# nintendops/EPN_PointCloud

Measured on AMD Instinct MI355X. Metric: point-clouds/sec fwd+bwd, ModelNet40 N=1024 A=60, higher is better.
Workload: dtype f32

## Files before the change

epn_pointcloud_amd/csrc/c_api.hip:

```cpp
#include <atomic>
#include <cstdlib>
#include <cstring>
#include <cxxabi.h>

#include "conv_internal.h"

using namespace epn;

static std::atomic<int> g_policy{0};
static bool force_generic() { return g_policy.load(std::memory_order_relaxed) == 1; }

namespace epn {
bool first_layer_on_valu() { return g_policy.load(std::memory_order_relaxed) == 2; }
#ifdef EPN_TUNING
int kernel_policy() { return g_policy.load(std::memory_order_relaxed); }
#else
int kernel_policy() { return 0; }
#endif
}

namespace {
thread_local const void *t_stub = nullptr;
thread_local bool t_stub_aux = true;
}
namespace epn {
void note_kernel(const void *host_stub, bool aux) {
    if (aux && t_stub) return;
    t_stub = host_stub;
    t_stub_aux = aux;
}
}

extern "C" const char *epn_last_kernel(void) {
    static thread_local char out[320];
    out[0] = 0;
    const void *stub = t_stub;
    t_stub = nullptr;
    t_stub_aux = true;
    if (!stub) return out;
    const char *mangled = hipKernelNameRefByPtr(stub, nullptr);
    if (!mangled) return out;
    int status = 0;
    char *dem = abi::__cxa_demangle(mangled, nullptr, nullptr, &status);
    const char *b = (status == 0 && dem) ? dem : mangled;
    if (!std::strncmp(b, "void ", 5)) b += 5;
    static const char anon[] = "(anonymous namespace)::";
    size_t o = 0;
    int depth = 0;
    for (size_t i = 0; b[i] && o + 1 < sizeof(out);) {
        if (!std::strncmp(b + i, anon, sizeof(anon) - 1)) { i += sizeof(anon) - 1; continue; }
        if (b[i] == '<') ++depth;
        else if (b[i] == '>') --depth;
        else if (b[i] == '(' && depth == 0) break;
        out[o++] = b[i++];
    }
    out[o] = 0;
    std::free(dem);
    return out;
}

extern "C" int epn_set_kernel_policy(int policy) {
#ifdef EPN_TUNING
    if (policy != 0 && policy != 1 && policy != 2 && (policy & ~0xff) != 0x100 && (policy & ~0xff) != 0x200 && (policy & ~0xff) != 0x400 && (policy & ~0xff) != 0x800 && (policy & ~0xff) != 0x900) return EPN_EINVAL;
#else
    if (policy != 0 && policy != 1 && policy != 2) return EPN_EINVAL;
#endif
    g_policy.store(policy, std::memory_order_relaxed);
    return 0;
}

static int check_desc(const epn_inter_desc *d) {
    if (!d) return EPN_ENULL;
    if (d->b < 0 || d->p1 < 1 || d->p2 < 0 || d->nn < 1 || d->na < 1 || d->ks < 1 || d->cin < 1 || d->cout < 1)
        return EPN_EINVAL;
    if (d->ks > EPN_KS_GENERIC_MAX) return EPN_EINVAL;
    if (!(d->sigma > 0.f) && !d->dense_w) return EPN_EINVAL;
    if (!d->ball_idx) return EPN_ENULL;
    if (!d->dense_w && (!d->xyz || !d->new_xyz || !d->anchors || !d->kernels)) return EPN_ENULL;
    return 0;
}

static bool use_mfma(const epn_inter_desc *d) { return inter_uses_mfma(d) && !force_generic() && !d->dense_w; }

extern "C" const char *epn_version(void) { return "epn_so3conv 0.5 (gfx950)"; }
extern "C" int epn_abi_version(void) { return EPN_ABI_VERSION; }

extern "C" const char *epn_strerror(int code) {
    switch (code) {
        case 0: return "success";
        case EPN_EINVAL: return "epn: invalid size or unsupported shape";
        case EPN_EWORKSPACE: return "epn: workspace missing or too small";
        case EPN_ENULL: return "epn: required pointer is NULL";
        default: return code > 0 ? hipGetErrorString((hipError_t)code) : "epn: unknown error";
    }
}

extern "C" int epn_inter_is_fused(const epn_inter_desc *d) {
    return d && (use_mfma(d) || (inter_c1_fwd_ok(d) && !force_generic())) ? 1 : 0;
// ... 480 lines not shown
```

epn_pointcloud_amd/csrc/gemm.h:

```cpp
#pragma once
#include "epn_common.h"

namespace epn {

constexpr int GEMM_MAX_PROB = 6;

struct GemmNtProb {
    const void *A, *Bt;
    void *C;
    long long M, lda, ldb, ldc;
    int N, K;
    int tiles_n;
    unsigned tile0;
    unsigned ntile;
    const void *Bp;
    float *stats;
    const float *a_amax, *b_amax;
    unsigned *c_amax;
};
struct GemmNtBatch {
    int nprob;
    unsigned ntiles;
    GemmNtProb p[GEMM_MAX_PROB];
};
// ... 21 lines not shown
        if (rc) return rc;
    }
    return 0;
}

inline unsigned nt_plan_tiles(GemmNtBatch &B, int BM, int BN) {
    for (int i = 1; i < B.nprob; ++i)
        for (int k = i; k > 0 && B.p[k].K > B.p[k - 1].K; --k) {
            const GemmNtProb tmp = B.p[k]; B.p[k] = B.p[k - 1]; B.p[k - 1] = tmp;
        }
    unsigned total = 0;
    for (int i = 0; i < B.nprob; ++i) {
        GemmNtProb &p = B.p[i];
        p.tiles_n = (p.N + BN - 1) / BN;
        p.tile0 = total;
        p.ntile = (unsigned)((p.M + BM - 1) / BM) * p.tiles_n;
        total += i + 1 < B.nprob ? (p.ntile + 7u) & ~7u : p.ntile;
    }
    B.ntiles = total;
    return total;
}

struct GemmTnArgs {
    const void *X, *Y;
    void *C, *part;
    size_t part_bytes;
    long long R, ldx, ldy, ldc;
    int N1, N2;
    unsigned ntiles;
    int tiles_n2, nsplit;
    unsigned block0;
    const void *Xp;
    const float *x_amax, *y_amax;
};
struct GemmTnBatch {
    int nprob;
    unsigned nblocks;
    GemmTnArgs p[GEMM_MAX_PROB];
};

#ifdef __HIPCC__
typedef __attribute__((address_space(3))) void lds_void;
typedef __attribute__((address_space(1))) const void glb_void;
typedef __bf16 bf16x8 __attribute__((ext_vector_type(8)));
typedef __bf16 bf16x4 __attribute__((ext_vector_type(4)));
typedef __bf16 bf16x2 __attribute__((ext_vector_type(2)));
typedef short s16x4 __attribute__((ext_vector_type(4)));
typedef float f32x2 __attribute__((ext_vector_type(2)));
typedef unsigned u32x4 __attribute__((ext_vector_type(4)));

template <typename T> struct ElemOf;
template <> struct ElemOf<float> { static constexpr int PER16 = 4; };
template <> struct ElemOf<__bf16> { static constexpr int PER16 = 8; };

__device__ __forceinline__ void glds16(const void *g, char *lds_wave_base) {
    __builtin_amdgcn_global_load_lds((glb_void *)g, (lds_void *)lds_wave_base, 16, 0, 0);
}

#define EPN_WAVE_UMAX(m_)                                                                       \
    _Pragma("unroll") for (int o = 32; o >= 1; o >>= 1) {                                        \
        const unsigned v = (unsigned)__shfl_xor((int)(m_), o, 64);                               \
        (m_) = v > (m_) ? v : (m_);                                                              \
    }
__device__ __forceinline__ unsigned absmax_finite(unsigned m, unsigned bits) {
    const unsigned a = bits & 0x7fffffffu;
    return (a > m && a < 0x7f800000u) ? a : m;
// ... 181 lines not shown
            const int n = col0 + 32 * j + li;
            if (lj == 0 && n < N) {
                float2 *o = reinterpret_cast<float2 *>(part + (((size_t)(rb >> 5)) * N + n) * 2);
                *o = make_float2(s1, s2);
            }
        }
    }
}
#endif

#ifdef __HIPCC__
template <int TM, int TN, typename TO>
__device__ __forceinline__ void nt_c_amax(const gemm_f32x16 (&acc)[TM][TN], unsigned *__restrict__ out) {
    float mf = 0.0f;
#pragma unroll
    for (int i = 0; i < TM; ++i)
#pragma unroll
        for (int j = 0; j < TN; ++j)
#pragma unroll
            for (int r = 0; r < 16; r += 2) mf = fmaxf(fmaxf(mf, fabsf(acc[i][j][r])), fabsf(acc[i][j][r + 1]));
    if constexpr (sizeof(TO) == 2) mf = (float)(__bf16)mf;
    unsigned m = __builtin_bit_cast(unsigned, mf);
    m = m < 0x7f800000u ? m : 0u;
    EPN_WAVE_UMAX(m)
    if ((threadIdx.x & 63) == 0 && m > __atomic_load_n(out, __ATOMIC_RELAXED)) atomicMax(out, m);
}
#endif

long long f2_nonfinite_take_gemm(bool reset);
long long f2_nonfinite_take_x3(bool reset);
long long f2_nonfinite_take_bwd(bool reset);

int kernel_policy();

int launch_gemm_nt(GemmNtBatch &B, int dtype, int out_dtype, hipStream_t st);
bool gemm_nt_x3_ok(const GemmNtBatch &B);
size_t gemm_nt_x3_workspace(const GemmNtBatch &B);
int launch_gemm_nt_x3(GemmNtBatch &B, void *ws, size_t ws_bytes, hipStream_t st, int npl = 3);
size_t gemm_nt_f2_workspace(const GemmNtBatch &B);
int launch_absmax(const float *src, long long ld, long long rows, long long cols, float *out, hipStream_t st);
int launch_scale_scalar(float *v, float factor, hipStream_t st, unsigned tag = 0);
int launch_absmax_unless_tagged(const float *src, long long n, float *slot, unsigned tag, hipStream_t st);
int launch_gemm_tn(GemmTnArgs &G, int dtype, hipStream_t st);
int launch_gemm_tn_batch(GemmTnBatch &B, int dtype, void *ws, size_t ws_bytes, hipStream_t st);
size_t gemm_tn_batch_workspace(GemmTnBatch &B, int dtype);
void gemm_tn_tile(int dtype, int N1, int N2, int *bn1, int *bn2);
int gemm_tn_splits(int dtype, long long R, int N1, int N2);
int launch_transpose_cast(const void *src, void *dst, int rows, int cols, int src_bf16, int dst_bf16, hipStream_t st);
int launch_cast(const void *src, void *dst, size_t n, int src_bf16, int dst_bf16, hipStream_t st);
int launch_cast_add(const float *src, const void *add_bf16, void *dst_bf16, size_t n, hipStream_t st);

}
```

epn_pointcloud_amd/csrc/gemm_tn.hip:

```cpp
#include "conv_internal.h"
#include "gemm.h"

namespace epn {
namespace {
EPN_F2_SENTINEL_DECL


#ifndef EPN_TN_GROUP_TARGET_BF16
#define EPN_TN_GROUP_TARGET_BF16 768
#endif
#ifndef EPN_TN_GROUP_TARGET_F32
#define EPN_TN_GROUP_TARGET_F32 1024
#endif
#ifndef EPN_TN_SINGLE_TARGET_BF16
#define EPN_TN_SINGLE_TARGET_BF16 512
#endif
#ifndef EPN_TN_SWZ
#define EPN_TN_SWZ 1
#endif
__device__ __forceinline__ int tn_row_swz(int r) { return 2 * ((r & 3) | (((r >> 3) & 1) << 2)); }
template <bool SWZ>
__device__ __forceinline__ int tn_swz_col(int col, int r) {
    if constexpr (!SWZ) return col;
    return (((col >> 3) ^ tn_row_swz(r)) << 3) | (col & 7);
}
#ifndef EPN_TN_WIDE_NSTG
#define EPN_TN_WIDE_NSTG 3
#endif
#ifndef EPN_TN_NARROW_NSTG
#define EPN_TN_NARROW_NSTG 4
#endif
#ifndef EPN_TN_NARROW_STAGE_KB
// ... 9 lines not shown
#define EPN_TN_NARROW_WGS 1
#endif
__device__ __forceinline__ unsigned tn_tile_of(unsigned lb, unsigned ntiles, unsigned nsplit) {
    return epn_xcd_tile(lb, (ntiles * nsplit + 7u) & ~7u);
}

template <int W, int K>
__device__ __forceinline__ void tn_frag_k(const char *p, float (&v)[W][K], int k) {
    static_assert(W == 1 || W == 2 || W == 4, "fragment width");
    if constexpr (W == 4) {
        const f32x4 q = *reinterpret_cast<const f32x4 *>(p);
        v[0][k] = q[0]; v[1][k] = q[1]; v[2][k] = q[2]; v[3][k] = q[3];
    } else if constexpr (W == 2) {
        const f32x2 q = *reinterpret_cast<const f32x2 *>(p);
        v[0][k] = q[0]; v[1][k] = q[1];
    } else {
        v[0][k] = *reinterpret_cast<const float *>(p);
    }
}
template <int W>
__device__ __forceinline__ void tn_frag(const char *p, float (&v)[W]) {
    static_assert(W == 1 || W == 2 || W == 4, "fragment width");
    if constexpr (W == 4) {
        const f32x4 q = *reinterpret_cast<const f32x4 *>(p);
        v[0] = q[0]; v[1] = q[1]; v[2] = q[2]; v[3] = q[3];
    } else if constexpr (W == 2) {
        const f32x2 q = *reinterpret_cast<const f32x2 *>(p);
        v[0] = q[0]; v[1] = q[1];
    } else {
        v[0] = *reinterpret_cast<const float *>(p);
    }
}

template <int WGM, int WGN, int TM, int TN, int BR, int X3 = 0>
__global__ __launch_bounds__(64 * WGM * WGN) void gemm_tn_f32_kernel(GemmTnBatch B) {
    constexpr int NW = WGM * WGN;
    constexpr int BN1 = WGM * TM * 32, BN2 = WGN * TN * 32;
    constexpr int ROWF = BN1 + BN2;
    constexpr int STAGE_B = BR * ROWF * 4;
    constexpr int NI = STAGE_B / 1024;
    constexpr int IPW = (NI + NW - 1) / NW;
    static_assert(STAGE_B % 1024 == 0, "stage must be a whole number of 1 KiB pieces");
    __shared__ __attribute__((aligned(1024))) char smem[2 * STAGE_B];

    const int lane = threadIdx.x & 63;
    const int wave = __builtin_amdgcn_readfirstlane(threadIdx.x >> 6);
    int pi = 0;
#pragma unroll
    for (int i = 1; i < GEMM_MAX_PROB; ++i)
        if (i < B.nprob && blockIdx.x >= B.p[i].block0) pi = i;
    const GemmTnArgs &G = B.p[pi];
    const unsigned tile = tn_tile_of(blockIdx.x - G.block0, G.ntiles, (unsigned)G.nsplit) % G.ntiles;
    const unsigned split = tn_tile_of(blockIdx.x - G.block0, G.ntiles, (unsigned)G.nsplit) / G.ntiles;
    if (split >= (unsigned)G.nsplit) return;
    const int n1_0 = (int)(tile / G.tiles_n2) * BN1, n2_0 = (int)(tile % G.tiles_n2) * BN2;
    const long long nchunk = G.R / BR;
    const long long c0 = nchunk * split / G.nsplit, c1 = nchunk * (split + 1) / G.nsplit;
    const int nk = (int)(c1 - c0);
    const float *__restrict__ X = static_cast<const float *>(G.X);
    const float *__restrict__ Y = static_cast<const float *>(G.Y);

    const float *src[IPW];
    long long sstep[IPW];
#pragma unroll
    for (int i = 0; i < IPW; ++i) {
        const int q = wave + i * NW;
// ... 91 lines not shown
                    const int g0 = (i * (NGRP - 1)) / IPW;
                    const int g1 = g0 + 1 < NGRP ? g0 + 1 : NGRP - 1;
                    if ((g0 == s && wpar == 0) || (g1 == s && wpar != 0)) stage_one((kt + 1) & 1, i);
                }
            }
            __builtin_amdgcn_sched_barrier(0);
#pragma unroll
            for (int i = 0; i < TM; ++i)
#pragma unroll
                for (int j = 0; j < TN; ++j)
                    acc[i][j] = __builtin_amdgcn_mfma_f32_32x32x2f32(a[s & 1][i], b[s & 1][j], acc[i][j], 0, 0, 0);
        }
    }

    if constexpr (X3 == 2) {
        const float ux = f2_inverse(x_scale), uy = f2_inverse(y_scale);
        EPN_F2_CHECK(f2_unscale(acc, ux, uy));
    }
    float *__restrict__ C = G.nsplit > 1 ? static_cast<float *>(G.part) + (size_t)split * G.N1 * G.N2
                                         : static_cast<float *>(G.C);
    const long long ldc = G.nsplit > 1 ? G.N2 : G.ldc;
    if (n1_0 + BN1 <= G.N1 && n2_0 + BN2 <= G.N2 && (long long)BN1 * ldc < (1LL << 30)) {
        float *__restrict__ cw = C + (size_t)(n1_0 + wm * TM * 32) * ldc + (n2_0 + wn * TN * 32);
        const unsigned ld = (unsigned)ldc;
        const unsigned lane_off = (unsigned)(TM * 4 * lj) * ld + TN * li;
#pragma unroll
        for (int i = 0; i < TM; ++i)
#pragma unroll
            for (int r = 0; r < 16; ++r) {
                const unsigned o = lane_off + (unsigned)(TM * ((r & 3) + 8 * (r >> 2)) + i) * ld;
#pragma unroll
                for (int j = 0; j < TN; ++j) cw[o + j] = acc[i][j][r];
            }
        return;
    }
#pragma unroll
    for (int i = 0; i < TM; ++i)
#pragma unroll
        for (int r = 0; r < 16; ++r) {
            const int ri = (r & 3) + 8 * (r >> 2) + 4 * lj;
            const int n1 = n1_0 + wm * TM * 32 + TM * ri + i;
            const int n2 = n2_0 + wn * TN * 32 + TN * li;
            if (n1 < G.N1) {
#pragma unroll
                for (int j = 0; j < TN; ++j)
                    if (n2 + j < G.N2) C[(long long)n1 * ldc + n2 + j] = acc[i][j][r];
            }
        }
}

__global__ void split_octets_kernel(const float *__restrict__ X, long long ldx, long long R, int N1, u32x4 *__restrict__ planes) {
    const long long i = (long long)blockIdx.x * blockDim.x + threadIdx.x;
    const long long n = (R >> 3) * N1;
    if (i >= n) return;
    const long long o = i / N1;
    const int c = (int)(i - o * N1);
    float x[8];
#pragma unroll
    for (int k = 0; k < 8; ++k) x[k] = X[(8 * o + k) * ldx + c];
    bf16x8 h, m, l;
    split3(x, h, m, l);
    planes[i] = __builtin_bit_cast(u32x4, h);
    planes[n + i] = __builtin_bit_cast(u32x4, m);
    planes[2 * n + i] = __builtin_bit_cast(u32x4, l);
}

__global__ void split_octets2_kernel(const float *__restrict__ X, long long ldx, long long R, int N1, u32x4 *__restrict__ planes,
                                     const float *__restrict__ amax) {
    const long long i = (long long)blockIdx.x * blockDim.x + threadIdx.x;
    const long long n = (R >> 3) * N1;
    if (i >= n) return;
    const long long o = i / N1;
    const int c = (int)(i - o * N1);
    float x[8];
#pragma unroll
    for (int k = 0; k < 8; ++k) x[k] = X[(8 * o + k) * ldx + c];
    gemm_f16x8 h, l;
    f2_split8(x, f2_scale_of(*amax), h, l);
    planes[i] = __builtin_bit_cast(u32x4, h);
    planes[n + i] = __builtin_bit_cast(u32x4, l);
}
// ... 108 lines not shown
            gemm_f16x8 ah[TM], al[TM], bh[TN], bl[TN];
#pragma unroll
            for (int i = 0; i < TM; ++i) {
                const char *xp = base + (2 * s + lj) * (BN1 * 16) + xo + i * 512;
                ah[i] = *reinterpret_cast<const gemm_f16x8 *>(xp);
                al[i] = *reinterpret_cast<const gemm_f16x8 *>(xp + OCT * BN1 * 16);
            }
#pragma unroll
            for (int j = 0; j < TN; ++j) f2_split8(yb[j], y_scale, bh[j], bl[j]);
            f2_terms(acc, ah, al, bh, bl);
            }
        }
    }

    if constexpr (NPL == 2) {
        const float ux = f2_inverse(f2_scale_of(*G.x_amax)), uy = f2_inverse(y_scale);
        EPN_F2_CHECK(f2_unscale(acc, ux, uy));
    }
    float *__restrict__ C = G.nsplit > 1 ? static_cast<float *>(G.part) + (size_t)split * G.N1 * G.N2
                                         : static_cast<float *>(G.C);
    const long long ldc = G.nsplit > 1 ? G.N2 : G.ldc;
    if (n1_0 + BN1 <= G.N1 && n2_0 + BN2 <= G.N2 && (long long)BN1 * ldc < (1LL << 30)) {
        float *__restrict__ cw = C + (size_t)(n1_0 + wm * TM * 32) * ldc + (n2_0 + wn * TN * 32);
        const unsigned ld = (unsigned)ldc;
        const unsigned lane_off = (unsigned)(4 * lj) * ld + TN * li;
#pragma unroll
        for (int i = 0; i < TM; ++i)
#pragma unroll
            for (int r = 0; r < 16; ++r) {
                const unsigned o = lane_off + (unsigned)(32 * i + (r & 3) + 8 * (r >> 2)) * ld;
#pragma unroll
                for (int j = 0; j < TN; ++j) cw[o + j] = acc[i][j][r];
            }
        return;
    }
#pragma unroll
    for (int i = 0; i < TM; ++i)
#pragma unroll
        for (int r = 0; r < 16; ++r) {
            const int n1 = n1_0 + wm * TM * 32 + 32 * i + (r & 3) + 8 * (r >> 2) + 4 * lj;
            const int n2 = n2_0 + wn * TN * 32 + TN * li;
            if (n1 < G.N1) {
#pragma unroll
                for (int j = 0; j < TN; ++j)
                    if (n2 + j < G.N2) C[(long long)n1 * ldc + n2 + j] = acc[i][j][r];
            }
        }
}

template <int WGM, int WGN, int TM, int TN>
__global__ __launch_bounds__(64 * WGM * WGN) void gemm_tn_bf16_kernel(GemmTnBatch B) {
    constexpr int NW = WGM * WGN;
    constexpr int BR = 32;
    constexpr int BN1 = WGM * TM * 16, BN2 = WGN * TN * 16;
    constexpr int ROWE = BN1 + BN2;
    constexpr int STAGE_B = BR * ROWE * 2;
    constexpr int NI = STAGE_B / 1024;
    constexpr int IPW = (NI + NW - 1) / NW;
    static_assert(STAGE_B % 1024 == 0, "stage must be a whole number of 1 KiB pieces");
    __shared__ __attribute__((aligned(1024))) char smem[2 * STAGE_B];

    const int lane = threadIdx.x & 63;
    const int wave = __builtin_amdgcn_readfirstlane(threadIdx.x >> 6);
    int pi = 0;
#pragma unroll
    for (int i = 1; i < GEMM_MAX_PROB; ++i)
        if (i < B.nprob && blockIdx.x >= B.p[i].block0) pi = i;
    const GemmTnArgs &G = B.p[pi];
    const unsigned tile = tn_tile_of(blockIdx.x - G.block0, G.ntiles, (unsigned)G.nsplit) % G.ntiles;
    const unsigned split = tn_tile_of(blockIdx.x - G.block0, G.ntiles, (unsigned)G.nsplit) / G.ntiles;
    if (split >= (unsigned)G.nsplit) return;
    const int n1_0 = (int)(tile / G.tiles_n2) * BN1, n2_0 = (int)(tile % G.tiles_n2) * BN2;
    const long long nchunk = G.R / BR;
    const long long c0 = nchunk * split / G.nsplit, c1 = nchunk * (split + 1) / G.nsplit;
    const int nk = (int)(c1 - c0);
    const __bf16 *__restrict__ X = static_cast<const __bf16 *>(G.X);
    const __bf16 *__restrict__ Y = static_cast<const __bf16 *>(G.Y);

    constexpr bool SWZ = EPN_TN_SWZ && BN1 % 128 == 0 && BN2 % 128 == 0;
    const __bf16 *src[IPW];
// ... 63 lines not shown
                (__attribute__((address_space(3))) s16x4 *)(base + ((tr_row + 4) * ROWE + col) * 2));
            typedef short s16x8 __attribute__((ext_vector_type(8)));
            const s16x8 v = {lo[0], lo[1], lo[2], lo[3], hi[0], hi[1], hi[2], hi[3]};
            b[j] = __builtin_bit_cast(bf16x8, v);
        }
#pragma unroll
        for (int i = 0; i < TM; ++i)
#pragma unroll
            for (int j = 0; j < TN; ++j) {
                acc[i][j] = __builtin_amdgcn_mfma_f32_16x16x32_bf16(a[i], b[j], acc[i][j], 0, 0, 0);
                if (i == 0 && j == 0) {
                    __builtin_amdgcn_sched_barrier(0);
                    if (kt + 1 < nk) stage((kt + 1) & 1);
                    __builtin_amdgcn_sched_barrier(0);
                }
            }
    }

    float *__restrict__ C = G.nsplit > 1 ? static_cast<float *>(G.part) + (size_t)split * G.N1 * G.N2
                                         : static_cast<float *>(G.C);
    const long long ldc = G.nsplit > 1 ? G.N2 : G.ldc;
    if (n1_0 + BN1 <= G.N1 && n2_0 + BN2 <= G.N2 && (long long)BN1 * ldc < (1LL << 30)) {
        float *__restrict__ cw = C + (size_t)(n1_0 + wm * TM * 16) * ldc + (n2_0 + wn * TN * 16);
        const unsigned ld = (unsigned)ldc;
        const unsigned lane_off = (unsigned)(4 * lg) * ld + li;
#pragma unroll
        for (int i = 0; i < TM; ++i)
#pragma unroll
            for (int r = 0; r < 4; ++r) {
                const unsigned o = lane_off + (unsigned)(i * 16 + r) * ld;
#pragma unroll
                for (int j = 0; j < TN; ++j) cw[o + j * 16] = acc[i][j][r];
            }
        return;
    }
#pragma unroll
    for (int i = 0; i < TM; ++i)
#pragma unroll
        for (int j = 0; j < TN; ++j)
#pragma unroll
            for (int r = 0; r < 4; ++r) {
                const int n1 = n1_0 + (wm * TM + i) * 16 + 4 * lg + r;
                const int n2 = n2_0 + (wn * TN + j) * 16 + li;
                if (n1 < G.N1 && n2 < G.N2) C[(long long)n1 * ldc + n2] = acc[i][j][r];
            }
}

template <int WGM, int WGN, int TM, int TN, int NSTG, int KR>
__global__ __launch_bounds__(64 * WGM * WGN) void gemm_tn_bf16_ring_kernel(GemmTnBatch B) {
    constexpr int NW = WGM * WGN;
    constexpr int BN1 = WGM * TM * 16, BN2 = WGN * TN * 16;
    constexpr int ROWE = BN1 + BN2;
    constexpr int BR = 32 * KR;
    constexpr int STAGE_B = BR * ROWE * 2;
    constexpr int NI = STAGE_B / 1024;
    constexpr int IPW = (NI + NW - 1) / NW;
    static_assert(STAGE_B % 1024 == 0, "stage must be a whole number of 1 KiB pieces");
    static_assert(NSTG >= 3 && NSTG <= 4 && NSTG * STAGE_B <= 160 * 1024, "ring of 3 or 4 stages in LDS");
    static_assert(IPW * (NSTG - 2) <= 63, "vmcnt range");
    __shared__ __attribute__((aligned(1024))) char smem[NSTG * STAGE_B];

    const int lane = threadIdx.x & 63;
    const int wave = __builtin_amdgcn_readfirstlane(threadIdx.x >> 6);
    int pi = 0;
#pragma unroll
    for (int i = 1; i < GEMM_MAX_PROB; ++i)
        if (i < B.nprob && blockIdx.x >= B.p[i].block0) pi = i;
    const GemmTnArgs &G = B.p[pi];
    const unsigned tile = tn_tile_of(blockIdx.x - G.block0, G.ntiles, (unsigned)G.nsplit) % G.ntiles;
    const unsigned split = tn_tile_of(blockIdx.x - G.block0, G.ntiles, (unsigned)G.nsplit) / G.ntiles;
    if (split >= (unsigned)G.nsplit) return;
    const int n1_0 = (int)(tile / G.tiles_n2) * BN1, n2_0 = (int)(tile % G.tiles_n2) * BN2;
    const long long nchunk = G.R / 32;
    const long long c0 = nchunk * split / G.nsplit, c1 = nchunk * (split + 1) / G.nsplit;
    const int nk = (int)(c1 - c0);
    const int nst = (nk + KR - 1) / KR;
    const __bf16 *__restrict__ X = static_cast<const __bf16 *>(G.X);
    const __bf16 *__restrict__ Y = static_cast<const __bf16 *>(G.Y);
// ... 78 lines not shown
                        b[j] = __builtin_bit_cast(bf16x8, v);
                    }
                }
                asm volatile("" : "+v"(lo[TN + i]), "+v"(hi[TN + i]));
                const s16x8 va = {lo[TN + i][0], lo[TN + i][1], lo[TN + i][2], lo[TN + i][3],
                                  hi[TN + i][0], hi[TN + i][1], hi[TN + i][2], hi[TN + i][3]};
                const bf16x8 a = __builtin_bit_cast(bf16x8, va);
#pragma unroll
                for (int j = 0; j < TN; ++j) {
                    acc[i][j] = __builtin_amdgcn_mfma_f32_16x16x32_bf16(a, b[j], acc[i][j], 0, 0, 0);
                    if (ks == 0 && i == 0 && j == 0) {
                        __builtin_amdgcn_sched_barrier(0);
                        if (kt + NSTG - 1 < nst) stage((kt + NSTG - 1) % NSTG);
                        __builtin_amdgcn_sched_barrier(0);
                    }
                }
            }
        }
    }

    float *__restrict__ C = G.nsplit > 1 ? static_cast<float *>(G.part) + (size_t)split * G.N1 * G.N2
                                         : static_cast<float *>(G.C);
    const long long ldc = G.nsplit > 1 ? G.N2 : G.ldc;
#pragma unroll
    for (int i = 0; i < TM; ++i)
#pragma unroll
        for (int j = 0; j < TN; ++j)
#pragma unroll
            for (int r = 0; r < 4; ++r) {
                const int n1 = n1_0 + (wm * TM + i) * 16 + 4 * lg + r;
                const int n2 = n2_0 + (wn * TN + j) * 16 + li;
                if (n1 < G.N1 && n2 < G.N2) C[(long long)n1 * ldc + n2] = acc[i][j][r];
            }
}

__global__ __launch_bounds__(256) void gemm_tn_reduce_kernel(GemmTnBatch B) {
    const GemmTnArgs &G = B.p[blockIdx.y];
    if (G.nsplit <= 1) return;
    const float *__restrict__ part = static_cast<const float *>(G.part);
    float *__restrict__ C = static_cast<float *>(G.C);
    const size_t n = (size_t)G.N1 * G.N2;
    const size_t stride = (size_t)gridDim.x * blockDim.x;
    if ((G.N2 & 3) == 0 && (G.ldc & 3) == 0 && !((uintptr_t)C & 15)) {
        const size_t n4 = n >> 2;
        for (size_t i = (size_t)blockIdx.x * blockDim.x + threadIdx.x; i < n4; i += stride) {
            const f32x4 *p = reinterpret_cast<const f32x4 *>(part) + i;
            f32x4 a[8];
#pragma unroll
            for (int u = 0; u < 8; ++u) a[u] = f32x4{0.f, 0.f, 0.f, 0.f};
            int k = 0;
            for (; k + 8 <= G.nsplit; k += 8)
#pragma unroll
                for (int u = 0; u < 8; ++u) {
                    const f32x4 v = p[(size_t)(k + u) * n4];
                    a[u][0] += v[0]; a[u][1] += v[1]; a[u][2] += v[2]; a[u][3] += v[3];
                }
            for (; k < G.nsplit; ++k) {
                const f32x4 v = p[(size_t)k * n4];
                a[0][0] += v[0]; a[0][1] += v[1]; a[0][2] += v[2]; a[0][3] += v[3];
            }
            f32x4 r;
#pragma unroll
            for (int e = 0; e < 4; ++e)
                r[e] = ((a[0][e] + a[1][e]) + (a[2][e] + a[3][e])) + ((a[4][e] + a[5][e]) + (a[6][e] + a[7][e]));
            const size_t e0 = i << 2;
            *reinterpret_cast<f32x4 *>(C + (e0 / G.N2) * G.ldc + (e0 % G.N2)) = r;
        }
        return;
    }
    for (size_t i = (size_t)blockIdx.x * blockDim.x + threadIdx.x; i < n; i += stride) {
        float s = 0.f;
        for (int k = 0; k < G.nsplit; ++k) s += part[(size_t)k * n + i];
        C[(i / G.N2) * G.ldc + (i % G.N2)] = s;
    }
}

template <int SP>
__global__ __launch_bounds__(256) void gemm_tn_reduce_sp_kernel(GemmTnBatch B) {
    constexpr int QB = 256 / SP;
    __shared__ f32x4 red[SP][QB];
    const GemmTnArgs &G = B.p[blockIdx.y];
    if (G.nsplit <= 1) return;
    const f32x4 *__restrict__ part = static_cast<const f32x4 *>(G.part);
    float *__restrict__ C = static_cast<float *>(G.C);
    const size_t n4 = ((size_t)G.N1 * G.N2) >> 2;
    const int ql = threadIdx.x % QB, g = threadIdx.x / QB;
    for (size_t q0 = (size_t)blockIdx.x * QB; q0 < n4; q0 += (size_t)gridDim.x * QB) {
        const size_t q = q0 + ql;
        f32x4 a[4];
#pragma unroll
        for (int u = 0; u < 4; ++u) a[u] = f32x4{0.f, 0.f, 0.f, 0.f};
        if (q < n4) {
            int k = g;
            for (; k + 3 * SP < G.nsplit; k += 4 * SP)
#pragma unroll
                for (int u = 0; u < 4; ++u) {
                    const f32x4 v = part[(size_t)(k + u * SP) * n4 + q];
                    a[u][0] += v[0]; a[u][1] += v[1]; a[u][2] += v[2]; a[u][3] += v[3];
                }
            for (; k < G.nsplit; k += SP) {
                const f32x4 v = part[(size_t)k * n4 + q];
                a[0][0] += v[0]; a[0][1] += v[1]; a[0][2] += v[2]; a[0][3] += v[3];
            }
        }
        f32x4 r;
#pragma unroll
        for (int e = 0; e < 4; ++e) r[e] = (a[0][e] + a[1][e]) + (a[2][e] + a[3][e]);
        red[g][ql] = r;
        __syncthreads();
        if (g == 0 && q < n4) {
            for (int j = 1; j < SP; ++j) {
                const f32x4 v = red[j][ql];
                r[0] += v[0]; r[1] += v[1]; r[2] += v[2]; r[3] += v[3];
            }
            const size_t e0 = q << 2;
            *reinterpret_cast<f32x4 *>(C + (e0 / G.N2) * G.ldc + (e0 % G.N2)) = r;
        }
        __syncthreads();
    }
}

template <typename T>
__global__ void gemm_tn_generic_kernel(const T *__restrict__ X, const T *__restrict__ Y, float *__restrict__ C,
                                       long long R, int N1, int N2, long long ldx, long long ldy, long long ldc) {
    const long long i = (long long)blockIdx.x * blockDim.x + threadIdx.x;
    if (i >= (long long)N1 * N2) return;
    const int n1 = (int)(i / N2), n2 = (int)(i % N2);
    float s = 0.f;
    for (long long r = 0; r < R; ++r) s = fmaf((float)X[r * ldx + n1], (float)Y[r * ldy + n2], s);
    C[(long long)n1 * ldc + n2] = s;
}

enum TnFamily { TN_F32, TN_PLANES, TN_BF16, TN_RING };
#define EPN_TN_F32_INSTANCES(X)                                                                                      \
    X(1, 8, 1, 2, 32)                                                                                 \
    X(2, 2, 1, 1, 32)                                                                                 \
    X(2, 2, 1, 2, 32)                                                                                 \
    X(1, 8, 2, 1, 32)                                                                                 \
    X(1, 4, 2, 4, 16)                                                                                 \
    X(2, 2, 2, 1, 32)                                                                                 \
    X(2, 2, 2, 2, 32)                                                                                 \
    X(2, 4, 2, 2, 32)                                                                                 \
    X(1, 8, 4, 2, 32)
#define EPN_TN_PLANES_INSTANCES(X)                                                                                   \
    X(1, 8, 1, 2, 32)                                                                                 \
    X(1, 8, 2, 2, 16)                                                                                 \
    X(2, 4, 2, 2, 32)                                   \
// ... 118 lines not shown
    }
    if (B.nprob == 1) {
        B.p[0].nsplit = gemm_tn_splits(bf, B.p[0].R, B.p[0].N1, B.p[0].N2);
    } else {
        const long long target = bf == 1 ? EPN_TN_GROUP_TARGET_BF16 : EPN_TN_GROUP_TARGET_F32;
        long long S = 8;
        for (long long cand = 8; cand <= 8192; ++cand) {
            long long blocks = 0;
            for (int i = 0; i < B.nprob; ++i) blocks += tiles[i] * ((chunks[i] + cand - 1) / cand);
            S = cand;
            if (blocks <= target) break;
        }
        for (int i = 0; i < B.nprob; ++i) {
            long long sp = (chunks[i] + S - 1) / S;
            sp = sp < 1 ? 1 : (sp > 512 ? 512 : sp);
            B.p[i].nsplit = (int)sp;
        }
    }
    size_t off = 0;
    unsigned blk = 0;
    for (int i = 0; i < B.nprob; ++i) {
        GemmTnArgs &G = B.p[i];
        G.block0 = blk;
        blk += (G.ntiles * (unsigned)G.nsplit + 7u) & ~7u;
        G.part = nullptr; G.part_bytes = 0;
        if (G.nsplit > 1) {
            const size_t nb = (size_t)G.nsplit * G.N1 * G.N2 * sizeof(float);
            if (ws) G.part = static_cast<char *>(ws) + off;
            G.part_bytes = nb;
            off += (nb + 255) & ~(size_t)255;
        }
    }
    B.nblocks = blk;
    for (int i = 0; i < B.nprob; ++i) B.p[i].Xp = nullptr;
    const bool planes = x3 && tn_has_instance(TN_PLANES, bn1, bn2) && tn_planes_form(B.nprob, min2, x3);
    if (planes)
        for (int i = 0; i < B.nprob; ++i) {
            GemmTnArgs &G = B.p[i];
            G.Xp = ws ? static_cast<char *>(ws) + off : reinterpret_cast<const void *>(1);
            off += ((size_t)2 * x3 * G.R * G.N1 + 255) & ~(size_t)255;
        }
    size_t amax_off = 0;
    if (x3 == 2) {
        amax_off = off;
        off += 256;
    }
    TnFamily family = planes ? TN_PLANES : TN_F32;
    if constexpr (sizeof(T) == 2) family = (B.nprob == 1 ? bn2 <= 128 : bn1 == 128) ? TN_RING : TN_BF16;
    return TnChoice{family, bn1, bn2, planes, off, amax_off};
}

template <typename T>
int launch_tn_typed(GemmTnBatch &B, void *ws, size_t ws_bytes, hipStream_t st, int x3 = 0) {
    bool fast = true;
    for (int i = 0; i < B.nprob; ++i) {
        const GemmTnArgs &G = B.p[i];
        if (G.R < 0 || G.N1 < 1 || G.N2 < 1) return EPN_EINVAL;
        if (!G.C) return EPN_ENULL;
        if (G.R > 0 && (!G.X || !G.Y)) return EPN_ENULL;
        fast = fast && tn_fast_ok<T>(G);
    }
    if (!fast) {
        for (int i = 0; i < B.nprob; ++i) {
            const GemmTnArgs &G = B.p[i];
            const long long n = (long long)G.N1 * G.N2;
            EPN_LAUNCH((gemm_tn_generic_kernel<T>), dim3((unsigned)((n + 255) / 256)), dim3(256), 0, st,
                               static_cast<const T *>(G.X), static_cast<const T *>(G.Y), static_cast<float *>(G.C), G.R,
                               G.N1, G.N2, G.ldx, G.ldy, G.ldc);
            EPN_CHECK_LAUNCH();
        }
        return 0;
    }
    const TnChoice ch = tn_plan<T>(B, ws, x3);
    if (ch.ws_bytes > 0 && (!ws || ws_bytes < ch.ws_bytes)) return EPN_EWORKSPACE;
    if (!tn_has_instance(ch.family, ch.bn1, ch.bn2)) return EPN_EINVAL;
    if constexpr (sizeof(T) == 4) {
        if (x3 == 2) {
            float *slots = reinterpret_cast<float *>(static_cast<char *>(ws) + ch.amax_off);
            for (int i = 0; i < B.nprob; ++i) {
                GemmTnArgs &G = B.p[i];
                if (!G.x_amax) {
                    int rc = launch_absmax(static_cast<const float *>(G.X), G.ldx, G.R, G.N1, slots + 2 * i, st);
                    if (rc) return rc;
                    G.x_amax = slots + 2 * i;
                }
                if (!G.y_amax) {
                    int rc = launch_absmax(static_cast<const float *>(G.Y), G.ldy, G.R, G.N2, slots + 2 * i + 1, st);
                    if (rc) return rc;
                    G.y_amax = slots + 2 * i + 1;
                }
            }
        }
        if (ch.planes) {
            for (int i = 0; i < B.nprob; ++i) {
                const GemmTnArgs &G = B.p[i];
                const long long n = (G.R >> 3) * G.N1;
                if (x3 == 3)
                    EPN_LAUNCH_AUX(split_octets_kernel, dim3((unsigned)((n + 255) / 256)), dim3(256), 0, st,
                                   static_cast<const float *>(G.X), G.ldx, G.R, G.N1, static_cast<u32x4 *>(const_cast<void *>(G.Xp)));
                else
                    EPN_LAUNCH_AUX(split_octets2_kernel, dim3((unsigned)((n + 255) / 256)), dim3(256), 0, st,
                                   static_cast<const float *>(G.X), G.ldx, G.R, G.N1, static_cast<u32x4 *>(const_cast<void *>(G.Xp)), G.x_amax);
                EPN_CHECK_LAUNCH();
            }
        }
    }
    const int rc = launch_tn_instance<T>(ch, B, st, x3);
    if (rc) return rc;
    EPN_CHECK_LAUNCH();
    bool any_split = false;
    size_t nmax = 0;
    for (int i = 0; i < B.nprob; ++i) {
        any_split = any_split || B.p[i].nsplit > 1;
        const size_t n = (size_t)B.p[i].N1 * B.p[i].N2;
        nmax = n > nmax ? n : nmax;
    }
    if (any_split) {
        const size_t nv = (nmax + 3) / 4;
        bool quads = true;
        int smax = 1;
        for (int i = 0; i < B.nprob; ++i) {
            const GemmTnArgs &G = B.p[i];
            quads = quads && (G.N2 & 3) == 0 && (G.ldc & 3) == 0 && !((uintptr_t)G.C & 15);
            smax = G.nsplit > smax ? G.nsplit : smax;
        }
        int sp = 1;
        while (quads && sp < 64 && smax > 16 * sp && nv * B.nprob * sp * 4 <= (1u << 20)) sp *= 4;
        if (sp > 1) {
            const size_t qb = 256 / sp;
            const unsigned gx = (unsigned)((nv + qb - 1) / qb < 2048 ? (nv + qb - 1) / qb : 2048);
            if (sp == 4) EPN_LAUNCH_AUX(gemm_tn_reduce_sp_kernel<4>, dim3(gx, B.nprob), dim3(256), 0, st, B);
            else if (sp == 16) EPN_LAUNCH_AUX(gemm_tn_reduce_sp_kernel<16>, dim3(gx, B.nprob), dim3(256), 0, st, B);
            else EPN_LAUNCH_AUX(gemm_tn_reduce_sp_kernel<64>, dim3(gx, B.nprob), dim3(256), 0, st, B);
        } else {
            const unsigned gx = (unsigned)((nv + 255) / 256 < 2048 ? (nv + 255) / 256 : 2048);
            EPN_LAUNCH_AUX(gemm_tn_reduce_kernel, dim3(gx, B.nprob), dim3(256), 0, st, B);
        }
        EPN_CHECK_LAUNCH();
    }
    return 0;
}

}

EPN_F2_SENTINEL_TAKE(f2_nonfinite_take_gemm)

void gemm_tn_tile(int dtype, int N1, int N2, int *bn1, int *bn2) {
    if (dtype == 1) {
        if (N2 <= 128) {
            *bn2 = N2 <= 32 ? 32 : (N2 <= 64 ? 64 : 128);
            *bn1 = N1 <= 32 ? 32 : (N1 <= 64 ? 64 : (N1 <= 128 ? 128 : 256));
            if (*bn2 == 32 && *bn1 > 64) *bn1 = 64;
            return;
        }
        if (N1 <= 32) { *bn1 = 32; *bn2 = 256; }
        else if (N1 <= 64) { *bn1 = 64; *bn2 = 256; }
        else { *bn1 = 128; *bn2 = 256; }
    } else {
        if (dtype == 2 && N2 >= 512) {
            if (N1 <= 32) { *bn1 = 32; *bn2 = 512; }
// ... 128 lines not shown
```

Measured before the change: 546.9.

## Fuse split-K partial reduction into the TN GEMM via last-arriver tile counters

```diff
diff --git a/epn_pointcloud_amd/csrc/c_api.hip b/epn_pointcloud_amd/csrc/c_api.hip
--- a/epn_pointcloud_amd/csrc/c_api.hip
+++ b/epn_pointcloud_amd/csrc/c_api.hip
@@ -12,6 +12,10 @@
 
 namespace epn {
 bool first_layer_on_valu() { return g_policy.load(std::memory_order_relaxed) == 2; }
+int tn_reduce_policy() {
+    const int p = g_policy.load(std::memory_order_relaxed);
+    return p == 3 || p == 4 ? p : 0;
+}
 #ifdef EPN_TUNING
 int kernel_policy() { return g_policy.load(std::memory_order_relaxed); }
 #else
@@ -61,9 +65,9 @@
 
 extern "C" int epn_set_kernel_policy(int policy) {
 #ifdef EPN_TUNING
-    if (policy != 0 && policy != 1 && policy != 2 && (policy & ~0xff) != 0x100 && (policy & ~0xff) != 0x200 && (policy & ~0xff) != 0x400 && (policy & ~0xff) != 0x800 && (policy & ~0xff) != 0x900) return EPN_EINVAL;
+    if ((policy < 0 || policy > 4) && (policy & ~0xff) != 0x100 && (policy & ~0xff) != 0x200 && (policy & ~0xff) != 0x400 && (policy & ~0xff) != 0x800 && (policy & ~0xff) != 0x900) return EPN_EINVAL;
 #else
-    if (policy != 0 && policy != 1 && policy != 2) return EPN_EINVAL;
+    if (policy < 0 || policy > 4) return EPN_EINVAL;
 #endif
     g_policy.store(policy, std::memory_order_relaxed);
     return 0;
diff --git a/epn_pointcloud_amd/csrc/gemm.h b/epn_pointcloud_amd/csrc/gemm.h
--- a/epn_pointcloud_amd/csrc/gemm.h
+++ b/epn_pointcloud_amd/csrc/gemm.h
@@ -77,6 +77,8 @@
     unsigned block0;
     const void *Xp;
     const float *x_amax, *y_amax;
+    unsigned *cnt;
+    int red_sp;
 };
 struct GemmTnBatch {
     int nprob;
@@ -324,6 +326,7 @@
 long long f2_nonfinite_take_bwd(bool reset);
 
 int kernel_policy();
+int tn_reduce_policy();
 
 int launch_gemm_nt(GemmNtBatch &B, int dtype, int out_dtype, hipStream_t st);
 bool gemm_nt_x3_ok(const GemmNtBatch &B);
diff --git a/epn_pointcloud_amd/csrc/gemm_tn.hip b/epn_pointcloud_amd/csrc/gemm_tn.hip
--- a/epn_pointcloud_amd/csrc/gemm_tn.hip
+++ b/epn_pointcloud_amd/csrc/gemm_tn.hip
@@ -1,3 +1,5 @@
+#include <atomic>
+
 #include "conv_internal.h"
 #include "gemm.h"
 
@@ -73,6 +75,131 @@
     }
 }
 
+__device__ __forceinline__ f32x4 tn_sum_rounds8(const f32x4 *__restrict__ p, size_t n4, int nsplit) {
+    f32x4 a[8];
+#pragma unroll
+    for (int u = 0; u < 8; ++u) a[u] = f32x4{0.f, 0.f, 0.f, 0.f};
+    int k = 0;
+    for (; k + 8 <= nsplit; k += 8)
+#pragma unroll
+        for (int u = 0; u < 8; ++u) {
+            const f32x4 v = p[(size_t)(k + u) * n4];
+            a[u][0] += v[0]; a[u][1] += v[1]; a[u][2] += v[2]; a[u][3] += v[3];
+        }
+    for (; k < nsplit; ++k) {
+        const f32x4 v = p[(size_t)k * n4];
+        a[0][0] += v[0]; a[0][1] += v[1]; a[0][2] += v[2]; a[0][3] += v[3];
+    }
+    f32x4 r;
+#pragma unroll
+    for (int e = 0; e < 4; ++e)
+        r[e] = ((a[0][e] + a[1][e]) + (a[2][e] + a[3][e])) + ((a[4][e] + a[5][e]) + (a[6][e] + a[7][e]));
+    return r;
+}
+__device__ __forceinline__ float tn_sum_serial(const float *__restrict__ p, size_t n, int nsplit) {
+    float s = 0.f;
+    for (int k = 0; k < nsplit; ++k) s += p[(size_t)k * n];
+    return s;
+}
+template <int SP>
+__device__ __forceinline__ f32x4 tn_sum_strided(const f32x4 *__restrict__ p, size_t n4, int g, int nsplit) {
+    f32x4 a[4];
+#pragma unroll
+    for (int u = 0; u < 4; ++u) a[u] = f32x4{0.f, 0.f, 0.f, 0.f};
+    int k = g;
+    for (; k + 3 * SP < nsplit; k += 4 * SP)
+#pragma unroll
+        for (int u = 0; u < 4; ++u) {
+            const f32x4 v = p[(size_t)(k + u * SP) * n4];
+            a[u][0] += v[0]; a[u][1] += v[1]; a[u][2] += v[2]; a[u][3] += v[3];
+        }
+    for (; k < nsplit; k += SP) {
+        const f32x4 v = p[(size_t)k * n4];
+        a[0][0] += v[0]; a[0][1] += v[1]; a[0][2] += v[2]; a[0][3] += v[3];
+    }
+    f32x4 r;
+#pragma unroll
+    for (int e = 0; e < 4; ++e) r[e] = (a[0][e] + a[1][e]) + (a[2][e] + a[3][e]);
+    return r;
+}
+template <int SP>
+__device__ __forceinline__ f32x4 tn_sum_combine(f32x4 r, const f32x4 *red, int qb, int ql) {
+    for (int j = 1; j < SP; ++j) {
+        const f32x4 v = red[j * qb + ql];
+        r[0] += v[0]; r[1] += v[1]; r[2] += v[2]; r[3] += v[3];
+    }
+    return r;
+}
+__device__ __forceinline__ bool tn_sum_quads(const GemmTnArgs &G) {
+    return (G.N2 & 3) == 0 && (G.ldc & 3) == 0 && !((uintptr_t)G.C & 15);
+}
+
+constexpr unsigned TN_ARRIVAL_POOL = 1u << 17;
+__device__ unsigned g_tn_arrivals[TN_ARRIVAL_POOL];
+
+template <int SP, int NT>
+__device__ __forceinline__ void tn_tile_sum_sp(const GemmTnArgs &G, int n1_0, int n2_0, int nr, int qc, f32x4 *red) {
+    constexpr int QB = NT / SP;
+    const f32x4 *__restrict__ part = static_cast<const f32x4 *>(G.part);
+    float *__restrict__ C = static_cast<float *>(G.C);
+    const size_t n4 = ((size_t)G.N1 * G.N2) >> 2;
+    const int ql = threadIdx.x % QB, g = threadIdx.x / QB;
+    const int nq = nr * qc;
+    for (int q0 = 0; q0 < nq; q0 += QB) {
+        const int q = q0 + ql;
+        const int row = n1_0 + q / qc, col = n2_0 + 4 * (q % qc);
+        f32x4 r = f32x4{0.f, 0.f, 0.f, 0.f};
+        if (q < nq) r = tn_sum_strided<SP>(part + (((size_t)row * G.N2 + col) >> 2), n4, g, G.nsplit);
+        red[g * QB + ql] = r;
+        __syncthreads();
+        if (g == 0 && q < nq) *reinterpret_cast<f32x4 *>(C + (size_t)row * G.ldc + col) = tn_sum_combine<SP>(r, red, QB, ql);
+        __syncthreads();
+    }
+}
+
+template <int NT, int BN1, int BN2>
+__device__ __forceinline__ void tn_sum_in_launch(const GemmTnArgs &G, unsigned tile, int n1_0, int n2_0, char *smem) {
+    asm volatile("s_waitcnt vmcnt(0)" ::: "memory");
+    __syncthreads();
+    unsigned *arrived = reinterpret_cast<unsigned *>(smem);
+    if (threadIdx.x == 0) {
+        __builtin_amdgcn_fence(__ATOMIC_RELEASE, "agent");
+        *arrived = __hip_atomic_fetch_add(G.cnt + tile, 1u, __ATOMIC_RELAXED, __HIP_MEMORY_SCOPE_AGENT);
+    }
+    __syncthreads();
+    const bool last = *arrived == (unsigned)G.nsplit - 1u;
+    __syncthreads();
+    if (!last) return;
+    __builtin_amdgcn_fence(__ATOMIC_ACQUIRE, "agent");
+
+    const int nr = G.N1 - n1_0 < BN1 ? G.N1 - n1_0 : BN1;
+    const int nc = G.N2 - n2_0 < BN2 ? G.N2 - n2_0 : BN2;
+    const size_t n = (size_t)G.N1 * G.N2;
+    float *__restrict__ C = static_cast<float *>(G.C);
+    if (!tn_sum_quads(G)) {
+        const float *__restrict__ part = static_cast<const float *>(G.part);
+        for (int i = threadIdx.x; i < nr * nc; i += NT) {
+            const int row = n1_0 + i / nc, col = n2_0 + i % nc;
+            C[(size_t)row * G.ldc + col] = tn_sum_serial(part + (size_t)row * G.N2 + col, n, G.nsplit);
+        }
+    } else if (G.red_sp == 1) {
+        const f32x4 *__restrict__ part = static_cast<const f32x4 *>(G.part);
+        const int qc = nc >> 2;
+        for (int q = threadIdx.x; q < nr * qc; q += NT) {
+            const int row = n1_0 + q / qc, col = n2_0 + 4 * (q % qc);
+            *reinterpret_cast<f32x4 *>(C + (size_t)row * G.ldc + col) =
+                tn_sum_rounds8(part + (((size_t)row * G.N2 + col) >> 2), n >> 2, G.nsplit);
+        }
+    } else {
+        static_assert(NT % 64 == 0, "a whole number of quads per pass for SP <= 64");
+        f32x4 *red = reinterpret_cast<f32x4 *>(smem);
+        if (G.red_sp == 4) tn_tile_sum_sp<4, NT>(G, n1_0, n2_0, nr, nc >> 2, red);
+        else if (G.red_sp == 16) tn_tile_sum_sp<16, NT>(G, n1_0, n2_0, nr, nc >> 2, red);
+        else tn_tile_sum_sp<64, NT>(G, n1_0, n2_0, nr, nc >> 2, red);
+    }
+    if (threadIdx.x == 0) __hip_atomic_store(G.cnt + tile, 0u, __ATOMIC_RELAXED, __HIP_MEMORY_SCOPE_AGENT);
+}
+
 template <int WGM, int WGN, int TM, int TN, int BR, int X3 = 0>
 __global__ __launch_bounds__(64 * WGM * WGN) void gemm_tn_f32_kernel(GemmTnBatch B) {
     constexpr int NW = WGM * WGN;
@@ -230,8 +357,7 @@
 #pragma unroll
                 for (int j = 0; j < TN; ++j) cw[o + j] = acc[i][j][r];
             }
-        return;
-    }
+    } else {
 #pragma unroll
     for (int i = 0; i < TM; ++i)
 #pragma unroll
@@ -245,6 +371,9 @@
                     if (n2 + j < G.N2) C[(long long)n1 * ldc + n2 + j] = acc[i][j][r];
             }
         }
+    }
+    static_assert(STAGE_B >= 16 * 64 * NW, "stage holds the in-launch sum's partials");
+    if (G.cnt) tn_sum_in_launch<64 * NW, BN1, BN2>(G, tile, n1_0, n2_0, smem);
 }
 
 __global__ void split_octets_kernel(const float *__restrict__ X, long long ldx, long long R, int N1, u32x4 *__restrict__ planes) {
@@ -419,8 +548,7 @@
 #pragma unroll
                 for (int j = 0; j < TN; ++j) cw[o + j] = acc[i][j][r];
             }
-        return;
-    }
+    } else {
 #pragma unroll
     for (int i = 0; i < TM; ++i)
 #pragma unroll
@@ -433,6 +561,9 @@
                     if (n2 + j < G.N2) C[(long long)n1 * ldc + n2 + j] = acc[i][j][r];
             }
         }
+    }
+    static_assert(STAGE_B >= 16 * 64 * NW, "stage holds the in-launch sum's partials");
+    if (G.cnt) tn_sum_in_launch<64 * NW, BN1, BN2>(G, tile, n1_0, n2_0, smem);
 }
 
 template <int WGM, int WGN, int TM, int TN>
@@ -562,8 +693,7 @@
 #pragma unroll
                 for (int j = 0; j < TN; ++j) cw[o + j * 16] = acc[i][j][r];
             }
-        return;
-    }
+    } else {
 #pragma unroll
     for (int i = 0; i < TM; ++i)
 #pragma unroll
@@ -574,6 +704,9 @@
                 const int n2 = n2_0 + (wn * TN + j) * 16 + li;
                 if (n1 < G.N1 && n2 < G.N2) C[(long long)n1 * ldc + n2] = acc[i][j][r];
             }
+    }
+    static_assert(STAGE_B >= 16 * 64 * NW, "stage holds the in-launch sum's partials");
+    if (G.cnt) tn_sum_in_launch<64 * NW, BN1, BN2>(G, tile, n1_0, n2_0, smem);
 }
 
 template <int WGM, int WGN, int TM, int TN, int NSTG, int KR>
@@ -718,6 +851,8 @@
                 const int n2 = n2_0 + (wn * TN + j) * 16 + li;
                 if (n1 < G.N1 && n2 < G.N2) C[(long long)n1 * ldc + n2] = acc[i][j][r];
             }
+    static_assert(STAGE_B >= 16 * 64 * NW, "stage holds the in-launch sum's partials");
+    if (G.cnt) tn_sum_in_launch<64 * NW, BN1, BN2>(G, tile, n1_0, n2_0, smem);
 }
 
 __global__ __launch_bounds__(256) void gemm_tn_reduce_kernel(GemmTnBatch B) {
@@ -727,44 +862,23 @@
     float *__restrict__ C = static_cast<float *>(G.C);
     const size_t n = (size_t)G.N1 * G.N2;
     const size_t stride = (size_t)gridDim.x * blockDim.x;
-    if ((G.N2 & 3) == 0 && (G.ldc & 3) == 0 && !((uintptr_t)C & 15)) {
+    if (tn_sum_quads(G)) {
         const size_t n4 = n >> 2;
         for (size_t i = (size_t)blockIdx.x * blockDim.x + threadIdx.x; i < n4; i += stride) {
-            const f32x4 *p = reinterpret_cast<const f32x4 *>(part) + i;
-            f32x4 a[8];
-#pragma unroll
-            for (int u = 0; u < 8; ++u) a[u] = f32x4{0.f, 0.f, 0.f, 0.f};
-            int k = 0;
-            for (; k + 8 <= G.nsplit; k += 8)
-#pragma unroll
-                for (int u = 0; u < 8; ++u) {
-                    const f32x4 v = p[(size_t)(k + u) * n4];
-                    a[u][0] += v[0]; a[u][1] += v[1]; a[u][2] += v[2]; a[u][3] += v[3];
-                }
-            for (; k < G.nsplit; ++k) {
-                const f32x4 v = p[(size_t)k * n4];
-                a[0][0] += v[0]; a[0][1] += v[1]; a[0][2] += v[2]; a[0][3] += v[3];
-            }
-            f32x4 r;
-#pragma unroll
-            for (int e = 0; e < 4; ++e)
-                r[e] = ((a[0][e] + a[1][e]) + (a[2][e] + a[3][e])) + ((a[4][e] + a[5][e]) + (a[6][e] + a[7][e]));
+            const f32x4 r = tn_sum_rounds8(reinterpret_cast<const f32x4 *>(part) + i, n4, G.nsplit);
             const size_t e0 = i << 2;
             *reinterpret_cast<f32x4 *>(C + (e0 / G.N2) * G.ldc + (e0 % G.N2)) = r;
         }
         return;
     }
-    for (size_t i = (size_t)blockIdx.x * blockDim.x + threadIdx.x; i < n; i += stride) {
-        float s = 0.f;
-        for (int k = 0; k < G.nsplit; ++k) s += part[(size_t)k * n + i];
-        C[(i / G.N2) * G.ldc + (i % G.N2)] = s;
-    }
+    for (size_t i = (size_t)blockIdx.x * blockDim.x + threadIdx.x; i < n; i += stride)
+        C[(i / G.N2) * G.ldc + (i % G.N2)] = tn_sum_serial(part + i, n, G.nsplit);
 }
 
 template <int SP>
 __global__ __launch_bounds__(256) void gemm_tn_reduce_sp_kernel(GemmTnBatch B) {
     constexpr int QB = 256 / SP;
-    __shared__ f32x4 red[SP][QB];
+    __shared__ f32x4 red[SP * QB];
     const GemmTnArgs &G = B.p[blockIdx.y];
     if (G.nsplit <= 1) return;
     const f32x4 *__restrict__ part = static_cast<const f32x4 *>(G.part);
@@ -773,32 +887,12 @@
     const int ql = threadIdx.x % QB, g = threadIdx.x / QB;
     for (size_t q0 = (size_t)blockIdx.x * QB; q0 < n4; q0 += (size_t)gridDim.x * QB) {
         const size_t q = q0 + ql;
-        f32x4 a[4];
-#pragma unroll
-        for (int u = 0; u < 4; ++u) a[u] = f32x4{0.f, 0.f, 0.f, 0.f};
-        if (q < n4) {
-            int k = g;
-            for (; k + 3 * SP < G.nsplit; k += 4 * SP)
-#pragma unroll
-                for (int u = 0; u < 4; ++u) {
-                    const f32x4 v = part[(size_t)(k + u * SP) * n4 + q];
-                    a[u][0] += v[0]; a[u][1] += v[1]; a[u][2] += v[2]; a[u][3] += v[3];
-                }
-            for (; k < G.nsplit; k += SP) {
-                const f32x4 v = part[(size_t)k * n4 + q];
-                a[0][0] += v[0]; a[0][1] += v[1]; a[0][2] += v[2]; a[0][3] += v[3];
-            }
-        }
-        f32x4 r;
-#pragma unroll
-        for (int e = 0; e < 4; ++e) r[e] = (a[0][e] + a[1][e]) + (a[2][e] + a[3][e]);
-        red[g][ql] = r;
+        f32x4 r = f32x4{0.f, 0.f, 0.f, 0.f};
+        if (q < n4) r = tn_sum_strided<SP>(part + q, n4, g, G.nsplit);
+        red[g * QB + ql] = r;
         __syncthreads();
         if (g == 0 && q < n4) {
-            for (int j = 1; j < SP; ++j) {
-                const f32x4 v = red[j][ql];
-                r[0] += v[0]; r[1] += v[1]; r[2] += v[2]; r[3] += v[3];
-            }
+            r = tn_sum_combine<SP>(r, red, QB, ql);
             const size_t e0 = q << 2;
             *reinterpret_cast<f32x4 *>(C + (e0 / G.N2) * G.ldc + (e0 % G.N2)) = r;
         }
@@ -983,7 +1077,7 @@
         }
     }
     B.nblocks = blk;
-    for (int i = 0; i < B.nprob; ++i) B.p[i].Xp = nullptr;
+    for (int i = 0; i < B.nprob; ++i) { B.p[i].Xp = nullptr; B.p[i].cnt = nullptr; B.p[i].red_sp = 0; }
     const bool planes = x3 && tn_has_instance(TN_PLANES, bn1, bn2) && tn_planes_form(B.nprob, min2, x3);
     if (planes)
         for (int i = 0; i < B.nprob; ++i) {
@@ -999,6 +1093,33 @@
     TnFamily family = planes ? TN_PLANES : TN_F32;
     if constexpr (sizeof(T) == 2) family = (B.nprob == 1 ? bn2 <= 128 : bn1 == 128) ? TN_RING : TN_BF16;
     return TnChoice{family, bn1, bn2, planes, off, amax_off};
+}
+
+#ifndef EPN_TN_IN_LAUNCH_MAX_KB
+#define EPN_TN_IN_LAUNCH_MAX_KB 256
+#endif
+inline bool tn_sum_in_launch_rule(const GemmTnBatch &B) {
+    const int pol = tn_reduce_policy();
+    if (pol) return pol == 4;
+    size_t worst = 0;
+    for (int i = 0; i < B.nprob; ++i) {
+        const GemmTnArgs &G = B.p[i];
+        if (G.nsplit <= 1) continue;
+        const size_t tile_b = (size_t)G.N1 * G.N2 * sizeof(float) / G.ntiles * G.nsplit;
+        worst = tile_b > worst ? tile_b : worst;
+    }
+    return worst <= (size_t)EPN_TN_IN_LAUNCH_MAX_KB * 1024;
+}
+std::atomic<unsigned> g_tn_cursor{0};
+inline int tn_take_arrivals(unsigned n, unsigned **out) {
+    if (n > TN_ARRIVAL_POOL) return EPN_EINVAL;
+    void *base = nullptr;
+    if (hipGetSymbolAddress(&base, HIP_SYMBOL(g_tn_arrivals)) != hipSuccess || !base) return EPN_EINVAL;
+    unsigned cur = g_tn_cursor.load(std::memory_order_relaxed), start;
+    do start = cur + n > TN_ARRIVAL_POOL ? 0u : cur;
+    while (!g_tn_cursor.compare_exchange_weak(cur, start + n, std::memory_order_relaxed));
+    *out = static_cast<unsigned *>(base) + start;
+    return 0;
 }
 
 template <typename T>
@@ -1056,27 +1177,40 @@
             }
         }
     }
+    bool any_split = false;
+    size_t nmax = 0;
+    bool quads = true;
+    int smax = 1;
+    unsigned ncnt = 0;
+    for (int i = 0; i < B.nprob; ++i) {
+        const GemmTnArgs &G = B.p[i];
+        any_split = any_split || G.nsplit > 1;
+        const size_t n = (size_t)G.N1 * G.N2;
+        nmax = n > nmax ? n : nmax;
+        quads = quads && (G.N2 & 3) == 0 && (G.ldc & 3) == 0 && !((uintptr_t)G.C & 15);
+        smax = G.nsplit > smax ? G.nsplit : smax;
+        if (G.nsplit > 1) ncnt += G.ntiles;
+    }
+    const size_t nv = (nmax + 3) / 4;
+    int sp = 1;
+    while (quads && sp < 64 && smax > 16 * sp && nv * B.nprob * sp * 4 <= (1u << 20)) sp *= 4;
+    const bool in_launch = any_split && tn_sum_in_launch_rule(B);
+    if (in_launch) {
+        unsigned *pool = nullptr;
+        const int rc = tn_take_arrivals(ncnt, &pool);
+        if (rc) return rc;
+        for (int i = 0; i < B.nprob; ++i) {
+            GemmTnArgs &G = B.p[i];
+            if (G.nsplit <= 1) continue;
+            G.cnt = pool;
+            G.red_sp = sp;
+            pool += G.ntiles;
+        }
+    }
     const int rc = launch_tn_instance<T>(ch, B, st, x3);
     if (rc) return rc;
     EPN_CHECK_LAUNCH();
-    bool any_split = false;
-    size_t nmax = 0;
-    for (int i = 0; i < B.nprob; ++i) {
-        any_split = any_split || B.p[i].nsplit > 1;
-        const size_t n = (size_t)B.p[i].N1 * B.p[i].N2;
-        nmax = n > nmax ? n : nmax;
-    }
-    if (any_split) {
-        const size_t nv = (nmax + 3) / 4;
-        bool quads = true;
-        int smax = 1;
-        for (int i = 0; i < B.nprob; ++i) {
-            const GemmTnArgs &G = B.p[i];
-            quads = quads && (G.N2 & 3) == 0 && (G.ldc & 3) == 0 && !((uintptr_t)G.C & 15);
-            smax = G.nsplit > smax ? G.nsplit : smax;
-        }
-        int sp = 1;
-        while (quads && sp < 64 && smax > 16 * sp && nv * B.nprob * sp * 4 <= (1u << 20)) sp *= 4;
+    if (any_split && !in_launch) {
         if (sp > 1) {
             const size_t qb = 256 / sp;
             const unsigned gx = (unsigned)((nv + qb - 1) / qb < 2048 ? (nv + qb - 1) / qb : 2048);
```

Result: no change. 545.3 (-0.3%).
